# ShawnNew/Detectron2-CenterNet

Measured on AMD Instinct MI355X. Metric: images/sec at 512x512 (infer bs=64), higher is better.
Workload: dtype f16x3; 1 GPU; DLA-34 CenterNet eval forward+decode, 64x3x512x512 uint8 per GPU, 80 classes, K=100, random-init weights (BatchNorm statistics calibrated), DCN offsets ~N(0,1px), 100 detections per image post-processed; per_gpu_batch=64, global_batch=64, parallelism=replicas x1

## Files before the change

### detectron2-centernet_amd/csrc/conv_common.h

```cpp
#pragma once
#include "common.h"
#include <type_traits>
__device__ __forceinline__ int swz(int row) { return (0x78 >> (2 * ((row >> 2) & 3))) & 3; }

__device__ __forceinline__ bool tile_of_block(int nbx, int nby, int& m_tile, int& n_tile) {
  const int lin = blockIdx.x;
  const int xcd = lin & 7, sq = lin >> 3;
  const int mchunk = (nbx + 7) >> 3;
  n_tile = sq % nby;
  const int m_local = sq / nby;
  m_tile = xcd * mchunk + m_local;
  return m_local < mchunk && m_tile < nbx;
}

struct DcnSample {
  int off[4];
  float wt[4];
  float mask;
  f16 wm[4];
};

template <bool NM = false>
__device__ __forceinline__ void dcn_setup(const ConvArgs& a, bool row_ok, int pix_base, int hb, int wb,
                                          int tr, int ts, const float* omrow, DcnSample& sp) {
  sp.off[0] = sp.off[1] = sp.off[2] = sp.off[3] = -1;
// ... 95 lines not shown
#pragma unroll
        for (int j = 0; j < 4; ++j) { v0[j] = fmaxf(v0[j], 0.f); v1[j] = fmaxf(v1[j], 0.f); }
      } else if (a.act == CTDET_ACT_SIGMOID_CLAMP) {
#pragma unroll
        for (int j = 0; j < 4; ++j) {
          v0[j] = fminf(fmaxf(ctdet_sigmoid_exact(v0[j]), a.clamp_lo), a.clamp_hi);
          v1[j] = fminf(fmaxf(ctdet_sigmoid_exact(v1[j]), a.clamp_lo), a.clamp_hi);
        }
      }
      TOut* yp = (TOut*)a.y + (long)m * a.out_stride + c0;
      if constexpr (sizeof(TOut) == 2) {
        f16x8 o;
#pragma unroll
        for (int j = 0; j < 4; ++j) { o[j] = (f16)v0[j]; o[4 + j] = (f16)v1[j]; }
        *(f16x8*)yp = o;
      } else {
        *(f32x4*)yp = v0;
        *(f32x4*)(yp + 4) = v1;
      }
    }
  }
}

static __device__ __attribute__((aligned(16))) unsigned int g_zero_page[64];

template <int N>
__device__ __forceinline__ void wait_vmcnt() {
  asm volatile("s_waitcnt vmcnt(%0)" ::"n"(N) : "memory");
}

__device__ __forceinline__ void wait_lgkm0() { __builtin_amdgcn_s_waitcnt(0xC07F); }

__device__ __forceinline__ void gload2_sync(const float* p, float& v0, float& v1) {
  typedef float f32x2_ __attribute__((ext_vector_type(2)));
  f32x2_ v;
  asm volatile("global_load_dwordx2 %0, %1, off\n\ts_waitcnt vmcnt(0)" : "=&v"(v) : "v"(p) : "memory");
  v0 = v[0]; v1 = v[1];
}
__device__ __forceinline__ void gload4_sync_into(const float* p, f32x4& v) {
  asm volatile("global_load_dwordx4 %0, %1, off\n\ts_waitcnt vmcnt(0)" : "+v"(v) : "v"(p) : "memory");
}

__device__ __forceinline__ void dma16(const void* g, char* lds_wave_base) {
  const unsigned l = __builtin_amdgcn_readfirstlane((unsigned)(size_t)lds_wave_base);
  asm volatile("s_mov_b32 m0, %0\n\ts_nop 0\n\tglobal_load_lds_dwordx4 %1, off" ::"s"(l), "v"(g) : "memory", "m0");
}
// ... 51 lines not shown
```

### detectron2-centernet_amd/csrc/conv_f32.hip

```cpp
#include "conv_common.h"

template <int BP, int BC, int WP, int WC_, bool SP>
__global__ void __launch_bounds__(256) conv_f32_mfma_kernel(const ConvArgs a) {
  constexpr int KS = 16, EPV = 4;
  constexpr int TP = BP / WP / 16;
  constexpr int TC = BC / WC_ / 16;
  constexpr int A_LD = BP / 64;
  constexpr int BCL = BC < 64 ? 64 : BC;
  constexpr int B_LD = BCL / 64;
  constexpr int NLOAD = A_LD + B_LD;
  constexpr int STAGE = (BP + BCL) * 64;
  constexpr int NST = 3;
  static_assert(WP * WC_ == 4, "4 waves per workgroup");
  __shared__ __attribute__((aligned(16))) char smem[NST * STAGE];

  const int tid = threadIdx.x, lane = tid & 63;
  const int wave = __builtin_amdgcn_readfirstlane(tid >> 6);
  const int wp = wave / WC_, wc = wave % WC_;
  int m_tile, n_tile;
  if (!tile_of_block((a.M + BP - 1) / BP, a.Cout_pad / BC, m_tile, n_tile)) return;
  const int m0 = m_tile * BP, n0 = n_tile * BC;
  const float* __restrict__ x = (const float*)a.x;
  const float* __restrict__ w = (const float*)a.w;
  const float* zero = (const float*)g_zero_page;
// ... 104 lines not shown
    f32x4 wf[TC], pf[TP];
#pragma unroll
    for (int c = 0; c < TC; ++c) wf[c] = *(const f32x4*)(base + BP * 64 + (wc * 16 * TC + 16 * c) * 64 + frag_off);
#pragma unroll
    for (int p = 0; p < TP; ++p) pf[p] = *(const f32x4*)(base + (wp * 16 * TP + 16 * p) * 64 + frag_off);
    if constexpr (SP) {
#pragma unroll
      for (int p = 0; p < TP; ++p) mma_px<true, TC>(wf, pf[p], acc[p]);
    } else {
#pragma unroll
      for (int e = 0; e < 4; ++e)
#pragma unroll
        for (int p = 0; p < TP; ++p)
#pragma unroll
          for (int c = 0; c < TC; ++c)
            acc[p][c] = __builtin_amdgcn_mfma_f32_16x16x4f32(wf[c][e], pf[p][e], acc[p][c], 0, 0, 0);
    }
    st_c = st_c == NST - 1 ? 0 : st_c + 1;
    st_l = st_l == NST - 1 ? 0 : st_l + 1;
  }

  const int q = lane >> 4;
  const int cb = n0 + wc * 16 * TC;
#pragma unroll
  for (int p = 0; p < TP; ++p) {
    const int m = m0 + wp * 16 * TP + 16 * p + fr;
    if (m >= a.M) continue;
    epilogue_tiles<float, TC>(a, m, cb, q, acc[p]);
  }
}

template <int BP, int BC, int WP, int WC_, bool CAT, bool SP>
__global__ void __launch_bounds__(256, 2) conv_f32_uk_kernel(const ConvArgs a) {
  constexpr int KS = 16, EPV = 4;
  constexpr int TP = BP / WP / 16;
  constexpr int TC = BC / WC_ / 16;
  constexpr int A_LD = BP / 64;
  constexpr int BCL = BC < 64 ? 64 : BC;
  constexpr int B_LD = BCL / 64;
  constexpr int NLOAD = A_LD + B_LD;
  constexpr int STAGE = (BP + BCL) * 64;
  constexpr int NST = 3;
  static_assert(WP * WC_ == 4, "4 waves per workgroup");
  __shared__ __attribute__((aligned(16))) char smem[NST * STAGE];

  const int tid = threadIdx.x, lane = tid & 63;
  const int wave = __builtin_amdgcn_readfirstlane(tid >> 6);
  const int wp = wave / WC_, wc = wave % WC_;
  int m_tile, n_tile;
  if (!tile_of_block((a.M + BP - 1) / BP, a.Cout_pad / BC, m_tile, n_tile)) return;
  const int m0 = m_tile * BP, n0 = n_tile * BC;
  const float* zero = (const float*)g_zero_page;
// ... 101 lines not shown
    f32x4 wf[TC];
#pragma unroll
    for (int c = 0; c < TC; ++c) wf[c] = *(const f32x4*)(fragB + ST * STAGE + c * 1024);
#pragma unroll
    for (int p = 0; p < TP; ++p) {
      const f32x4 pf = *(const f32x4*)(fragA + ST * STAGE + p * 1024);
      mma_px<SP, TC>(wf, pf, acc[p]);
    }
  };
  using I0 = std::integral_constant<int, 0>;
  using I1 = std::integral_constant<int, 1>;
  using I2 = std::integral_constant<int, 2>;
  int kt = 0;
  for (; kt + 2 < nk; kt += 3) {
    kstep(kt, I0{}, I2{});
    kstep(kt + 1, I1{}, I0{});
    kstep(kt + 2, I2{}, I1{});
  }
  if (kt < nk) { kstep(kt, I0{}, I2{}); ++kt; }
  if (kt < nk) { kstep(kt, I1{}, I0{}); ++kt; }

  const int q = lane >> 4;
  const int cb = n0 + wc * 16 * TC;
#pragma unroll
  for (int p = 0; p < TP; ++p) {
    const int m = m0 + wp * 16 * TP + 16 * p + fr;
    if (m >= a.M) continue;
    epilogue_tiles<float, TC>(a, m, cb, q, acc[p]);
  }
}

template <int BP, int BC, int WP, int WC_, bool SP, bool NM = false>
__global__ void __launch_bounds__(256, 2) dcn_f32_mfma_kernel(const ConvArgs a) {
  constexpr int KS = 16, EPV = 4;
  constexpr int TP = BP / WP / 16;
  constexpr int TC = BC / WC_ / 16;
  constexpr int A_LD = BP / 64;
  constexpr int BCL = BC < 64 ? 64 : BC;
  constexpr int B_LD = BCL / 64;
  constexpr int ASTAGE = BP * 64, WSTAGE = BCL * 64;
  static_assert(WP * WC_ == 4, "4 waves per workgroup");
  __shared__ __attribute__((aligned(16))) char smem[2 * ASTAGE + 2 * WSTAGE];
  char* const smA = smem;
  char* const smW = smem + 2 * ASTAGE;

  const int tid = threadIdx.x, lane = tid & 63;
  const int wave = __builtin_amdgcn_readfirstlane(tid >> 6);
  const int wp = wave / WC_, wc = wave % WC_;
  int m_tile, n_tile;
  if (!tile_of_block((a.M + BP - 1) / BP, a.Cout_pad / BC, m_tile, n_tile)) return;
  const int m0 = m_tile * BP, n0 = n_tile * BC;
  const float* __restrict__ x = (const float*)a.x;
// ... 97 lines not shown
    const char* bW = smW + (kt & 1) * WSTAGE;
    f32x4 wf[TC], pf[TP];
#pragma unroll
    for (int c = 0; c < TC; ++c) wf[c] = *(const f32x4*)(bW + (wc * 16 * TC + 16 * c) * 64 + frag_off);
#pragma unroll
    for (int p = 0; p < TP; ++p) pf[p] = *(const f32x4*)(bA + (wp * 16 * TP + 16 * p) * 64 + frag_off);
    if constexpr (SP) {
#pragma unroll
      for (int p = 0; p < TP; ++p) mma_px<true, TC>(wf, pf[p], acc[p]);
    } else {
#pragma unroll
      for (int e = 0; e < 4; ++e)
#pragma unroll
        for (int p = 0; p < TP; ++p)
#pragma unroll
          for (int c = 0; c < TC; ++c)
            acc[p][c] = __builtin_amdgcn_mfma_f32_16x16x4f32(wf[c][e], pf[p][e], acc[p][c], 0, 0, 0);
    }
    if (more) blend_store(smA + ((kt + 1) & 1) * ASTAGE);
  }

  const int q = lane >> 4;
  const int cb = n0 + wc * 16 * TC;
#pragma unroll
  for (int p = 0; p < TP; ++p) {
    const int m = m0 + wp * 16 * TP + 16 * p + fr;
    if (m >= a.M) continue;
    epilogue_tiles<float, TC>(a, m, cb, q, acc[p]);
  }
}

template <int BC, bool SP, bool NM = false>
__global__ void __launch_bounds__(256, 2) dcn_f32_window_kernel(const ConvArgs a) {
  constexpr int TH = 8, TW = 16, BP = 128, MG = 4;
  constexpr int WR = TH + 2 + 2 * MG, WCOLS = TW + 2 + 2 * MG;
  constexpr int NPIECE = WR * WCOLS * 4;
  constexpr int W_LD = (NPIECE + 255) / 256;
  constexpr int WINB = ((NPIECE + 63) / 64) * 1024;
  constexpr int GEOB = 9 * BP * 16, GEOC = 9 * BP * 4;
  constexpr int TP = 2, TC = BC / 16;
  constexpr int B_LD = BC / 64, WST = BC * 64, NST = 2, STG = 3 * WST;
  static_assert(BC % 64 == 0 && WINB + GEOB + GEOC + NST * STG <= 81920, "two workgroups per CU");
  __shared__ __attribute__((aligned(16))) char smem[WINB + GEOB + GEOC + NST * STG];
  char* const win = smem;
  char* const geo = smem + WINB;
  char* const geoc = smem + WINB + GEOB;
  char* const ring = smem + WINB + GEOB + GEOC;

  const int tid = threadIdx.x, lane = tid & 63;
  const int wave = __builtin_amdgcn_readfirstlane(tid >> 6);
  const int tiles_x = a.W / TW, tiles_y = a.H / TH;
  int m_tile, n_tile;
// ... 171 lines not shown
      asm volatile("" ::: "memory");
      sample(0, chunk + 1, pfn);
    }
#pragma unroll
    for (int p = 0; p < TP; ++p) pf[p] = pfn[p];
    if (TS < 2) {
#pragma unroll
      for (int c = 0; c < TC; ++c) wf[c] = wfn[c];
    }
  };
  for (int chunk = 0; chunk < nch; ++chunk) {
    const int s = chunk * 3;
    tap(s, chunk, std::integral_constant<int, 0>{});
    tap(s, chunk, std::integral_constant<int, 1>{});
    tap(s, chunk, std::integral_constant<int, 2>{});
    tap(s + 1, chunk, std::integral_constant<int, 3>{});
    tap(s + 1, chunk, std::integral_constant<int, 4>{});
    tap(s + 1, chunk, std::integral_constant<int, 5>{});
    tap(s + 2, chunk, std::integral_constant<int, 6>{});
    tap(s + 2, chunk, std::integral_constant<int, 7>{});
    tap(s + 2, chunk, std::integral_constant<int, 8>{});
  }

#pragma unroll
  for (int p = 0; p < TP; ++p) {
    const int m = (b * a.H + ty0 + prow) * a.W + tx0 + 8 * p + pcol;
    epilogue_tiles<float, TC>(a, m, n0, q, acc[p]);
  }
}

template <int TP, int BC, bool COLS = false, bool NM = false, bool FUS = false>
__global__ void __launch_bounds__(512 / TP, (TP == 1 && BC == 64) ? 4 : 2) dcn_split_window_kernel(const ConvArgs a) {
  static_assert(!FUS || (TP == 2 && BC == 64 && !COLS && !NM), "the fused offset conv: inference form of the 64-cout DCNv2 tile");
  constexpr int TH = 8, TW = 16, BP = 128, MG = 4;
  constexpr int NT = 512 / TP;
  static_assert(BC * 4 <= NT, "at most one weight piece per thread and tap (waves beyond BC / 16 fetch none)");
  constexpr int WR = TH + 2 + 2 * MG, WCOLS = TW + 2 + 2 * MG;
  constexpr int NPIECE = WR * WCOLS * 4;
  constexpr int W_LD = (NPIECE + NT - 1) / NT;
  constexpr int WINB = ((NPIECE + 63) / 64) * 1024;
  constexpr int GEOW = 9 * BP * 16, GEOC = 9 * BP * 4;
  constexpr int TC = BC / 16;
  constexpr int WST = BC * 64, NST = 2, STG = 3 * WST;
  static_assert(WINB + GEOW + GEOC + NST * STG <= ((TP == 2 || BC == 64) ? 81920 : 163840), "two workgroups / one (128 couts) per CU");
  __shared__ __attribute__((aligned(16))) char smem[WINB + GEOW + GEOC + NST * STG];
  char* const win = smem;
  char* const geow = smem + WINB;
  char* const geoc = smem + WINB + GEOW;
  char* const ring = smem + WINB + GEOW + GEOC;

  const int tid = threadIdx.x, lane = tid & 63;
// ... 377 lines not shown
    if (T < 8) {
      blend(raw, b1, b2, T + 1, chunk);
    } else if (chunk + 1 < nch) {
      wait_vmcnt<0>();
      __builtin_amdgcn_s_barrier();
      asm volatile("" ::: "memory");
      gather(0, chunk + 1, raw);
      blend(raw, b1, b2, 0, chunk + 1);
    }
  };
  for (int chunk = 0; chunk < nch; ++chunk) {
    const int s = chunk * 3;
    tap(s, chunk, std::integral_constant<int, 0>{});
    tap(s, chunk, std::integral_constant<int, 1>{});
    tap(s, chunk, std::integral_constant<int, 2>{});
    tap(s + 1, chunk, std::integral_constant<int, 3>{});
    tap(s + 1, chunk, std::integral_constant<int, 4>{});
    tap(s + 1, chunk, std::integral_constant<int, 5>{});
    tap(s + 2, chunk, std::integral_constant<int, 6>{});
    tap(s + 2, chunk, std::integral_constant<int, 7>{});
    tap(s + 2, chunk, std::integral_constant<int, 8>{});
  }

#pragma unroll
  for (int p = 0; p < TP; ++p) {
    const int m = (b * a.H + ty0 + prow) * a.W + tx0 + (TP == 2 ? 8 * p : 0) + pcol;
    epilogue_tiles<float, TC>(a, m, n0, q, acc[p]);
  }
}

template <int R, int CIN, int TC, int STRIDE, int TH, bool NOCHECK, bool SP>
__global__ void __launch_bounds__(256) conv_f32_win_kernel(const ConvArgs a) {
  constexpr int TW = STRIDE == 1 ? 64 : 32;
  constexpr int WH = (TH - 1) * STRIDE + R, WW = (TW - 1) * STRIDE + R;
  constexpr int PB = CIN * 4;
  constexpr int PPR = WW * PB / 16;
  constexpr int NP = WH * PPR, ROUNDS = (NP + 255) / 256;
  constexpr int K = R * R * CIN, NK = (K + 15) / 16;
  constexpr int GPT = CIN / 4;
  constexpr int NT = TW / 16, RW = TH / 4;
  static_assert(TH % 4 == 0 && ROUNDS * 4096 <= 65536, "tile");
  __shared__ __attribute__((aligned(16))) char win[ROUNDS * 4096];

  const int tid = threadIdx.x, lane = tid & 63;
  const int wave = __builtin_amdgcn_readfirstlane(tid >> 6);
  const int fr = lane & 15, q = lane >> 4;
  const int tiles_x = a.Wo / TW, tiles_y = a.Ho / TH;
  const int tx0 = (blockIdx.x % tiles_x) * TW;
  const int ty0 = ((blockIdx.x / tiles_x) % tiles_y) * TH;
  const int b = blockIdx.x / (tiles_x * tiles_y);
  const float* zero = (const float*)g_zero_page;
// ... 72 lines not shown
        if constexpr (SP) {
          const f16x8 h0 = __builtin_bit_cast(f16x8, pf0), h1 = __builtin_bit_cast(f16x8, pf1);
#pragma unroll
          for (int c = 0; c < TC; ++c) {
            acc[0][c] = __builtin_amdgcn_mfma_f32_16x16x32_f16(wa[kt][c], h0, acc[0][c], 0, 0, 0);
            acc[1][c] = __builtin_amdgcn_mfma_f32_16x16x32_f16(wa[kt][c], h1, acc[1][c], 0, 0, 0);
          }
#pragma unroll
          for (int c = 0; c < TC; ++c) {
            acc[0][c] = __builtin_amdgcn_mfma_f32_16x16x32_f16(wb[kt][c], h0, acc[0][c], 0, 0, 0);
            acc[1][c] = __builtin_amdgcn_mfma_f32_16x16x32_f16(wb[kt][c], h1, acc[1][c], 0, 0, 0);
          }
        } else {
#pragma unroll
          for (int e = 0; e < 4; ++e)
#pragma unroll
            for (int c = 0; c < TC; ++c) {
              acc[0][c] = __builtin_amdgcn_mfma_f32_16x16x4f32(wf[kt][c][e], pf0[e], acc[0][c], 0, 0, 0);
              acc[1][c] = __builtin_amdgcn_mfma_f32_16x16x4f32(wf[kt][c][e], pf1[e], acc[1][c], 0, 0, 0);
            }
        }
      }
      const int m = (b * a.Ho + ty0 + wave * RW + rr) * a.Wo + tx0 + tc * 16 + fr;
      epilogue_tiles<float, TC>(a, m, 0, q, acc[0]);
      epilogue_tiles<float, TC>(a, m + 16, 0, q, acc[1]);
    }
  }
}

template <bool SP> static const char* sp_name() { return SP ? "f16x3" : "f32"; }

template <int R, int CIN, int TC, int STRIDE, int TH, bool SP>
static int launch_f32_win(const ConvArgs& a, hipStream_t s) {
  constexpr int TW = STRIDE == 1 ? 64 : 32;
  const int tiles = a.B * (a.Ho / TH) * (a.Wo / TW);
  CTDET_KERNEL("conv_%s_win_kernel<%dx%d,Cin%d,Cout%d,s%d>", sp_name<SP>(), R, R, CIN, 16 * TC, STRIDE);
  if (a.pad == 0)
    hipLaunchKernelGGL((conv_f32_win_kernel<R, CIN, TC, STRIDE, TH, true, SP>), dim3(tiles), dim3(256), 0, s, a);
  else
    hipLaunchKernelGGL((conv_f32_win_kernel<R, CIN, TC, STRIDE, TH, false, SP>), dim3(tiles), dim3(256), 0, s, a);
  CTDET_LAUNCH_CHECK();
  return 0;
}

template <bool DEFORM, bool SP, bool NM = false>
__global__ void __launch_bounds__(256) conv_direct_f32_kernel(const ConvArgs a) {
  const long idx = (long)blockIdx.x * 256 + threadIdx.x;
  const int CP = (a.Cout + 3) & ~3;
// ... 258 lines not shown
```

### detectron2-centernet_amd/csrc/conv_igemm.hip

```cpp
#include "common.h"
#include <type_traits>
#include <stdlib.h>

#include "conv_common.h"

template <int BP, int BC, int WP, int WC_, typename TOut>
__global__ void __launch_bounds__(256) conv_igemm_dma_kernel(const ConvArgs a) {
  constexpr int TP = BP / WP / 16;
  constexpr int TC = BC / WC_ / 16;
  constexpr int A_LD = BP / 64;
  constexpr int BCL = BC < 64 ? 64 : BC;
  constexpr int B_LD = BCL / 64;
  constexpr int NLOAD = A_LD + B_LD;
  constexpr int STAGE = (BP + BCL) * 64;
  constexpr int NST = 3;
  static_assert(WP * WC_ == 4, "4 waves per workgroup");
  __shared__ __attribute__((aligned(16))) char smem[NST * STAGE];

  const int tid = threadIdx.x, lane = tid & 63;
  const int wave = __builtin_amdgcn_readfirstlane(tid >> 6);
  const int wp = wave / WC_, wc = wave % WC_;
  int m_tile, n_tile;
  if (!tile_of_block((a.M + BP - 1) / BP, a.Cout_pad / BC, m_tile, n_tile)) return;
  const int m0 = m_tile * BP, n0 = n_tile * BC;
// ... 103 lines not shown

  int st_c = 0, st_l = 2;
  for (int kt = 0; kt < nk; ++kt) {
    if (kt + 1 < nk) wait_vmcnt<NLOAD>(); else wait_vmcnt<0>();
    asm volatile("s_waitcnt lgkmcnt(0)" ::: "memory");
    __builtin_amdgcn_s_barrier();
    if (kt + 2 < nk) { issue(kt + 2, st_l); advance_k(); }
    const char* base = smem + st_c * STAGE;
    f16x8 wf[TC];
#pragma unroll
    for (int c = 0; c < TC; ++c) wf[c] = *(const f16x8*)(base + BP * 64 + (wc * 16 * TC + 16 * c) * 64 + frag_off);
#pragma unroll
    for (int p = 0; p < TP; ++p) {
      const f16x8 pf = *(const f16x8*)(base + (wp * 16 * TP + 16 * p) * 64 + frag_off);
#pragma unroll
      for (int c = 0; c < TC; ++c) acc[p][c] = __builtin_amdgcn_mfma_f32_16x16x32_f16(wf[c], pf, acc[p][c], 0, 0, 0);
    }
    st_c = st_c == NST - 1 ? 0 : st_c + 1;
    st_l = st_l == NST - 1 ? 0 : st_l + 1;
  }

  const int q = lane >> 4;
  const int cb = n0 + wc * 16 * TC;
#pragma unroll
  for (int p = 0; p < TP; ++p) {
    const int m = m0 + wp * 16 * TP + 16 * p + fr;
    if (m >= a.M) continue;
    epilogue_tiles<TOut, TC>(a, m, cb, q, acc[p]);
  }
}

template <int BP, int BC, int WP, int WC_, bool CAT, typename TOut>
__global__ void __launch_bounds__(256, 2) conv_igemm_uk_kernel(const ConvArgs a) {
  constexpr int TP = BP / WP / 16;
  constexpr int TC = BC / WC_ / 16;
  constexpr int A_LD = BP / 64;
  constexpr int BCL = BC < 64 ? 64 : BC;
  constexpr int B_LD = BCL / 64;
  constexpr int NLOAD = A_LD + B_LD;
  constexpr int STAGE = (BP + BCL) * 64;
  constexpr int NST = 3;
  static_assert(WP * WC_ == 4, "4 waves per workgroup");
  __shared__ __attribute__((aligned(16))) char smem[NST * STAGE];

  const int tid = threadIdx.x, lane = tid & 63;
  const int wave = __builtin_amdgcn_readfirstlane(tid >> 6);
  const int wp = wave / WC_, wc = wave % WC_;
  int m_tile, n_tile;
  if (!tile_of_block((a.M + BP - 1) / BP, a.Cout_pad / BC, m_tile, n_tile)) return;
  const int m0 = m_tile * BP, n0 = n_tile * BC;
  const f16* zero = (const f16*)g_zero_page;
  asm volatile("" : "+v"(zero));
// ... 101 lines not shown
#pragma unroll
    for (int c = 0; c < TC; ++c) wf[c] = *(const f16x8*)(fragB + ST * STAGE + c * 1024);
#pragma unroll
    for (int p = 0; p < TP; ++p) {
      const f16x8 pf = *(const f16x8*)(fragA + ST * STAGE + p * 1024);
#pragma unroll
      for (int c = 0; c < TC; ++c) acc[p][c] = __builtin_amdgcn_mfma_f32_16x16x32_f16(wf[c], pf, acc[p][c], 0, 0, 0);
    }
  };
  using I0 = std::integral_constant<int, 0>;
  using I1 = std::integral_constant<int, 1>;
  using I2 = std::integral_constant<int, 2>;
  int kt = 0;
  for (; kt + 2 < nk; kt += 3) {
    kstep(kt, I0{}, I2{});
    kstep(kt + 1, I1{}, I0{});
    kstep(kt + 2, I2{}, I1{});
  }
  if (kt < nk) { kstep(kt, I0{}, I2{}); ++kt; }
  if (kt < nk) { kstep(kt, I1{}, I0{}); ++kt; }

  const int q = lane >> 4;
  const int cb = n0 + wc * 16 * TC;
#pragma unroll
  for (int p = 0; p < TP; ++p) {
    const int m = m0 + wp * 16 * TP + 16 * p + fr;
    if (m >= a.M) continue;
    epilogue_tiles<TOut, TC>(a, m, cb, q, acc[p]);
  }
}

template <int BC, int WP, int WC_, typename TOut, bool SP = false>
__global__ void __launch_bounds__(256, 2) conv3x3_halo_kernel(const ConvArgs a) {
  using TIn = std::conditional_t<SP, float, f16>;
  constexpr int CH = SP ? 16 : 32, EPV = SP ? 4 : 8;
  static_assert(!SP || std::is_same<TOut, float>::value, "split mode stores f32");
  constexpr int TH = 8, TW = 32, BP = TH * TW;
  constexpr int TP = BP / WP / 16;
  constexpr int TC = BC / WC_ / 16;
  constexpr int ROWS_W = TH / WP;
  constexpr int BCL = BC < 64 ? 64 : BC;
  constexpr int B_LD = BCL / 64;
  constexpr int HMAIN = 10 * 32 * 64, HSIDE = 4096, HBUF = HMAIN + HSIDE;
  constexpr int WST = BCL * 64;
  static_assert(WP * WC_ == 4 && TP == 2 * ROWS_W, "wave layout");
  __shared__ __attribute__((aligned(16))) char smem[2 * HBUF + 3 * WST];
  char* const ring = smem + 2 * HBUF;

  const int tid = threadIdx.x, lane = tid & 63;
  const int wave = __builtin_amdgcn_readfirstlane(tid >> 6);
  const int wp = wave / WC_, wc = wave % WC_;
  const int tiles_x = a.W / TW, tiles_y = a.H / TH;
// ... 107 lines not shown
      }
    }
  };
  auto chunk_steps = [&](int kt, int chunk, auto hbc) {
    kstep(kt + 0, chunk, std::integral_constant<int, 0>{}, hbc);
    kstep(kt + 1, chunk, std::integral_constant<int, 1>{}, hbc);
    kstep(kt + 2, chunk, std::integral_constant<int, 2>{}, hbc);
    kstep(kt + 3, chunk, std::integral_constant<int, 3>{}, hbc);
    kstep(kt + 4, chunk, std::integral_constant<int, 4>{}, hbc);
    kstep(kt + 5, chunk, std::integral_constant<int, 5>{}, hbc);
    kstep(kt + 6, chunk, std::integral_constant<int, 6>{}, hbc);
    kstep(kt + 7, chunk, std::integral_constant<int, 7>{}, hbc);
    kstep(kt + 8, chunk, std::integral_constant<int, 8>{}, hbc);
  };
  int chunk = 0;
  for (; chunk + 1 < nch; chunk += 2) {
    chunk_steps(chunk * 9, chunk, std::integral_constant<int, 0>{});
    chunk_steps(chunk * 9 + 9, chunk + 1, std::integral_constant<int, 1>{});
  }
  if (chunk < nch) chunk_steps(chunk * 9, chunk, std::integral_constant<int, 0>{});

  const int q = lane >> 4;
  const int cb = n0 + wc * 16 * TC;
#pragma unroll
  for (int p = 0; p < TP; ++p) {
    const int y = ty0 + row0 + (p >> 1), x = tx0 + 16 * (p & 1) + l15;
    const int m = (b * a.H + y) * a.W + x;
    epilogue_tiles<TOut, TC>(a, m, cb, q, acc[p]);
  }
}

template <int BC, int WP, int WC_, typename TOut, bool SP = false>
static int launch_halo(const ConvArgs& a, hipStream_t s) {
  const int nbx = a.B * (a.H / 8) * (a.W / 32), nby = a.Cout_pad / BC;
  dim3 grid(8 * ((nbx + 7) / 8) * nby);
  CTDET_KERNEL("conv3x3_halo_kernel<256x%d,%s>", BC, SP ? "f16x3" : out_name<TOut>());
  hipLaunchKernelGGL((conv3x3_halo_kernel<BC, WP, WC_, TOut, SP>), grid, dim3(256), 0, s, a);
  CTDET_LAUNCH_CHECK();
  return 0;
}

template <int BC, int WP, int WC_>
__global__ void __launch_bounds__(256, 2) conv3x3_halo_pair_kernel(const ConvArgs a) {
  constexpr int TH = 8, TW = 32, BP = TH * TW;
  constexpr int TP = BP / WP / 16;
  constexpr int TC = BC / WC_ / 16;
  constexpr int ROWS_W = TH / WP;
  constexpr int BCL = BC < 64 ? 64 : BC;
  constexpr int W_LD = BCL / 64;
  constexpr int HMAIN = 10 * 32 * 64, HSIDE = 4096, HBUF = HMAIN + HSIDE;
  constexpr int WIMG = BCL * 64, WST = 2 * WIMG, NST = 3;
  static_assert(WP * WC_ == 4 && TP == 2 * ROWS_W, "wave layout");
// ... 194 lines not shown
  };
  auto next_stage = [](int st) { return st == NST - 1 ? 0 : st + 1; };
  auto chunk_steps = [&](int chunk, int st0, auto hbc, auto p0c) {
    constexpr int P0 = decltype(p0c)::value;
    const int kt = chunk * 5;
    int st = st0;
    kstep(kt + 0, chunk, st, std::integral_constant<int, 0>{}, hbc, std::integral_constant<int, P0>{}); st = next_stage(st);
    kstep(kt + 1, chunk, st, std::integral_constant<int, 1>{}, hbc, std::integral_constant<int, P0 ^ 1>{}); st = next_stage(st);
    kstep(kt + 2, chunk, st, std::integral_constant<int, 2>{}, hbc, std::integral_constant<int, P0>{}); st = next_stage(st);
    kstep(kt + 3, chunk, st, std::integral_constant<int, 3>{}, hbc, std::integral_constant<int, P0 ^ 1>{}); st = next_stage(st);
    kstep(kt + 4, chunk, st, std::integral_constant<int, 4>{}, hbc, std::integral_constant<int, P0>{});
  };
  int chunk = 0, st0 = 0;
  for (; chunk + 1 < nch; chunk += 2) {
    chunk_steps(chunk, st0, std::integral_constant<int, 0>{}, std::integral_constant<int, 0>{});
    st0 = (st0 + 2) % 3;
    chunk_steps(chunk + 1, st0, std::integral_constant<int, 1>{}, std::integral_constant<int, 1>{});
    st0 = (st0 + 2) % 3;
  }
  if (chunk < nch) chunk_steps(chunk, st0, std::integral_constant<int, 0>{}, std::integral_constant<int, 0>{});

  const int q = lane >> 4;
  const int cb = n0 + wc * 16 * TC;
#pragma unroll
  for (int p = 0; p < TP; ++p) {
    const int y = ty0 + row0 + (p >> 1), x = tx0 + 16 * (p & 1) + l15;
    const int m = (b * a.H + y) * a.W + x;
    epilogue_tiles<float, TC>(a, m, cb, q, acc[p]);
  }
}

template <int BC>
constexpr int pair2_smem_bytes() {
  return 2 * (10 * 32 * 64 + 4096) + 3 * 2 * (BC < 64 ? 64 : BC) * 64;
}

template <int BC, int WP, int WC_, int TW>
__device__ __forceinline__ void pair2_kloop(const ConvArgs& a, char* smem, int b, int ty0, int tx0, int n0,
                                            f32x4 (&acc)[256 / WP / 16][BC / WC_ / 16]) {
  constexpr int TH = 256 / TW, BP = TH * TW;
  constexpr int EN = TW / 16;
  constexpr int RS = TW * 64;
  constexpr int RPR = 256 * 16 / RS;
  constexpr int TP = BP / WP / 16;
  constexpr int TC = BC / WC_ / 16;
  constexpr int ROWS_W = TH / WP;
  constexpr int BCL = BC < 64 ? 64 : BC;
  constexpr int W_LD = BCL / 64;
  constexpr int HMAIN = 10 * 32 * 64, HSIDE = 4096, HBUF = HMAIN + HSIDE;
  constexpr int WIMG = BCL * 64, WST = 2 * WIMG, NST = 3;
  static_assert(WP * WC_ == 4 && TP == EN * ROWS_W && (TH + 2 + RPR - 1) / RPR == 5, "wave layout");
  static_assert(2 * HBUF + NST * WST == pair2_smem_bytes<BC>(), "LDS layout");
// ... 203 lines not shown
    kstep(kt + 6, pair, std::integral_constant<int, 6>{});
    kstep(kt + 7, pair, std::integral_constant<int, 7>{});
    kstep(kt + 8, pair, std::integral_constant<int, 8>{});
  }
}

template <int BC, int WP, int WC_, int TW = 32>
__global__ void __launch_bounds__(256, BC > 64 ? 1 : 2) conv3x3_halo_pair2_kernel(const ConvArgs a) {
  constexpr int TH = 256 / TW, EN = TW / 16, TP = 256 / WP / 16, TC = BC / WC_ / 16, ROWS_W = TH / WP;
  __shared__ __attribute__((aligned(16))) char smem[pair2_smem_bytes<BC>()];
  const int tiles_x = a.W / TW, tiles_y = a.H / TH;
  int m_tile, n_tile;
  if (!tile_of_block(a.B * tiles_y * tiles_x, a.Cout_pad / BC, m_tile, n_tile)) return;
  const int tx0 = (m_tile % tiles_x) * TW;
  const int ty0 = ((m_tile / tiles_x) % tiles_y) * TH;
  const int b = m_tile / (tiles_x * tiles_y);
  const int n0 = n_tile * BC;
  f32x4 acc[TP][TC];
  pair2_kloop<BC, WP, WC_, TW>(a, smem, b, ty0, tx0, n0, acc);

  const int lane = threadIdx.x & 63, wave = __builtin_amdgcn_readfirstlane(threadIdx.x >> 6);
  const int row0 = (wave / WC_) * ROWS_W, l15 = lane & 15, q = lane >> 4;
  const int cb = n0 + (wave % WC_) * 16 * TC;
#pragma unroll
  for (int p = 0; p < TP; ++p) {
    const int y = ty0 + row0 + p / EN, x = tx0 + 16 * (p % EN) + l15;
    const int m = (b * a.H + y) * a.W + x;
    epilogue_tiles<float, TC>(a, m, cb, q, acc[p]);
  }
}

template <int BC, int WP, int WC_, typename TOut, int TW = 32>
__global__ void __launch_bounds__(256, 2) conv3x3_halo_tap2_kernel(const ConvArgs a) {
  constexpr int TH = 256 / TW, BP = TH * TW;
  constexpr int EN = TW / 16, RS = TW * 64, RPR = 256 * 16 / RS;
  constexpr int TP = BP / WP / 16;
  constexpr int TC = BC / WC_ / 16;
  constexpr int ROWS_W = TH / WP;
  constexpr int BCL = BC < 64 ? 64 : BC;
  constexpr int W_LD = BCL / 64;
  constexpr int HMAIN = 10 * 32 * 64, HSIDE = 4096, HBUF = HMAIN + HSIDE;
  constexpr int WIMG = BCL * 64, WST = 2 * WIMG, NST = 3;
  static_assert(WP * WC_ == 4 && TP == EN * ROWS_W && (TH + 2 + RPR - 1) / RPR == 5, "wave layout");
  static_assert(2 * HBUF + NST * WST <= 81920, "two workgroups per CU");
  __shared__ __attribute__((aligned(16))) char smem[2 * HBUF + NST * WST];
  char* const ring = smem + 2 * HBUF;

  const int tid = threadIdx.x, lane = tid & 63;
  const int wave = __builtin_amdgcn_readfirstlane(tid >> 6);
  const int wp = wave / WC_, wc = wave % WC_;
  const int tiles_x = a.W / TW, tiles_y = a.H / TH;
  int m_tile, n_tile;
// ... 161 lines not shown
#pragma unroll
      for (int i = 2 * sl; i < 2 * sl + 2; ++i) mfma1(Par{}, 2, i, 1, 0);
      __builtin_amdgcn_sched_barrier(0);
    }
    load_px1(2, NextS{}, 0);
    load_px1(3, NextS{}, 0);
    __builtin_amdgcn_sched_barrier(0);
  };
  for (int pair = 0; pair < npair; ++pair) {
    const int kt = pair * 9;
    kstep(kt + 0, pair, std::integral_constant<int, 0>{});
    kstep(kt + 1, pair, std::integral_constant<int, 1>{});
    kstep(kt + 2, pair, std::integral_constant<int, 2>{});
    kstep(kt + 3, pair, std::integral_constant<int, 3>{});
    kstep(kt + 4, pair, std::integral_constant<int, 4>{});
    kstep(kt + 5, pair, std::integral_constant<int, 5>{});
    kstep(kt + 6, pair, std::integral_constant<int, 6>{});
    kstep(kt + 7, pair, std::integral_constant<int, 7>{});
    kstep(kt + 8, pair, std::integral_constant<int, 8>{});
  }

  const int q = lane >> 4;
  const int cb = n0 + wc * 16 * TC;
#pragma unroll
  for (int p = 0; p < TP; ++p) {
    const int y = ty0 + row0 + p / EN, x = tx0 + 16 * (p % EN) + l15;
    const int m = (b * a.H + y) * a.W + x;
    epilogue_tiles<TOut, TC>(a, m, cb, q, acc[p]);
  }
}

template <int BC, int WP, int WC_>
static int launch_halo_pair_t(const ConvArgs& a, hipStream_t s) {
  const int nbx = a.B * (a.H / 8) * (a.W / 32), nby = a.Cout_pad / BC;
  dim3 grid(8 * ((nbx + 7) / 8) * nby);
  CTDET_KERNEL("conv3x3_halo_pair_kernel<256x%d,f16x3>", BC);
  hipLaunchKernelGGL((conv3x3_halo_pair_kernel<BC, WP, WC_>), grid, dim3(256), 0, s, a);
  CTDET_LAUNCH_CHECK();
  return 0;
}

template <int BC, int WP, int WC_, int TW = 32>
static int launch_halo_pair2_t(const ConvArgs& a, hipStream_t s) {
  const int nbx = a.B * (a.H / (256 / TW)) * (a.W / TW), nby = a.Cout_pad / BC;
  dim3 grid(8 * ((nbx + 7) / 8) * nby);
  CTDET_KERNEL(TW == 32 ? "conv3x3_halo_pair2_kernel<256x%d,f16x3>" : "conv3x3_halo_pair2_kernel<16x16x%d,f16x3>", BC);
  hipLaunchKernelGGL((conv3x3_halo_pair2_kernel<BC, WP, WC_, TW>), grid, dim3(256), 0, s, a);
  CTDET_LAUNCH_CHECK();
  return 0;
}

template <int BC, int WP, int WC_, typename TOut, int TW = 32>
// ... 287 lines not shown
    pair2_kloop<BC, WP, 1, TW>(c, smem, b, ty0, tx0, n0, acc);

    f16x8 hf[TP][TC / 2], lf[TP][TC / 2];
#pragma unroll
    for (int hb = 0; hb < TC / 2; ++hb) {
      const int c0 = n0 + hb * 32 + q * 8;
      const f32x4 sa = *(const f32x4*)(a.s1 + c0), sb = *(const f32x4*)(a.s1 + c0 + 4);
      const f32x4 ba = *(const f32x4*)(a.b1 + c0), bb = *(const f32x4*)(a.b1 + c0 + 4);
#pragma unroll
      for (int p = 0; p < TP; ++p) {
        const f32x4 v0 = acc[p][2 * hb] * sa + ba, v1 = acc[p][2 * hb + 1] * sb + bb;
        f16x8 hi, lo;
#pragma unroll
        for (int j = 0; j < 8; ++j) {
          const float h = fmaxf(j < 4 ? v0[j] : v1[j - 4], 0.f);
          hi[j] = (f16)h;
          lo[j] = (f16)(h - (float)hi[j]);
        }
        hf[p][hb] = hi;
        lf[p][hb] = lo;
      }
    }
    for (int ot = 0; ot < ntile2; ++ot) {
      f32x4 o[TP];
#pragma unroll
      for (int p = 0; p < TP; ++p) o[p] = (f32x4){0.f, 0.f, 0.f, 0.f};
      const f16* wrow = w2 + (long)(ot * 16 + l15) * (2 * HID) + sl * BC + q * 8;
#pragma unroll
      for (int hb = 0; hb < TC / 2; ++hb) {
        const f16x8 X = *(const f16x8*)(wrow + hb * 32), Y = *(const f16x8*)(wrow + HID + hb * 32);
#pragma unroll
        for (int p = 0; p < TP; ++p) o[p] = __builtin_amdgcn_mfma_f32_16x16x32_f16(X, hf[p][hb], o[p], 0, 0, 0);
#pragma unroll
        for (int p = 0; p < TP; ++p) o[p] = __builtin_amdgcn_mfma_f32_16x16x32_f16(Y, hf[p][hb], o[p], 0, 0, 0);
#pragma unroll
        for (int p = 0; p < TP; ++p) o[p] = __builtin_amdgcn_mfma_f32_16x16x32_f16(X, lf[p][hb], o[p], 0, 0, 0);
      }
      const int c0 = ot * 16 + 4 * q;
      if (c0 < cw) {
#pragma unroll
        for (int p = 0; p < TP; ++p) {
          float* yp = yh + mpix[p] * ystride + c0;
          f32x4 v = o[p];
          if (sl > 0) v = *(const f32x4*)yp + v;
          if (sl == NSL - 1) {
            v = v * *(const f32x4*)(b2 + rows2 + c0) + *(const f32x4*)(b2 + c0);
            if (act == CTDET_ACT_RELU) {
#pragma unroll
              for (int j = 0; j < 4; ++j) v[j] = fmaxf(v[j], 0.f);
            } else if (act == CTDET_ACT_SIGMOID_CLAMP) {
#pragma unroll
              for (int j = 0; j < 4; ++j) v[j] = fminf(fmaxf(ctdet_sigmoid_exact(v[j]), a.clamp_lo), a.clamp_hi);
            }
          }
          *(f32x4*)yp = v;
        }
      }
    }
  }
}

int launch_head_fused_x3(const HeadArgs& a, hipStream_t s) {
  CTDET_CHECK(a.nheads >= 1 && a.nheads <= 4, "head_fused_x3: 1..4 heads");
  CTDET_CHECK(head_fused_x_ok(a, true) && (((size_t)a.w1 | (size_t)a.s1 | (size_t)a.b1) & 15) == 0,
              "head_fused_x3: needs Cin %% 32 == 0 and a map divisible by 8x32 or 16x16 (Cin=%d, %dx%d)", a.Cin, a.H, a.W);
  for (int h = 0; h < a.nheads; ++h)
    CTDET_CHECK(a.cout[h] >= 1 && a.cout[h] <= 256 && a.y_stride[h] % 4 == 0 && a.y_stride[h] >= ((a.cout[h] + 3) & ~3) &&
                    ((((size_t)a.y[h]) | (size_t)a.w2[h] | (size_t)a.b2[h]) & 15) == 0,
                "head_fused_x3: head %d: bad output (cout %d, stride %d)", h, a.cout[h], a.y_stride[h]);
// ... 1126 lines not shown
  for (int c = 0; c < TC; ++c) {
    const f16* wr = (const f16*)a.w + (long)cout_of<TC>(c, fr >> 2, fr & 3) * a.Kpad + q * 8;
#pragma unroll
    for (int kt = 0; kt < NK; ++kt) wf[kt][c] = *(const f16x8*)(wr + kt * 32);
  }
  int kaddr[NK];
#pragma unroll
  for (int kt = 0; kt < NK; ++kt) {
    const int G = kt * 4 + q;
    const int tap = G / GPT;
    const bool tail = tap >= R * R;
    const int tr = tail ? 0 : tap / R, ts = tail ? 0 : tap - (tap / R) * R;
    kaddr[kt] = ((wave * RW * STRIDE + tr) * WW + fr * STRIDE + ts) * PB + (tail ? 0 : (G - tap * GPT) * 16);
  }
  wait_vmcnt<0>();
  __syncthreads();

#pragma unroll
  for (int rr = 0; rr < RW; ++rr) {
#pragma unroll
    for (int tc = 0; tc < NT; ++tc) {
      constexpr int dummy = 0; (void)dummy;
      const int toff = (rr * STRIDE * WW + tc * 16 * STRIDE) * PB;
      f32x4 acc[TC];
#pragma unroll
      for (int c = 0; c < TC; ++c) acc[c] = (f32x4){0.f, 0.f, 0.f, 0.f};
#pragma unroll
      for (int kt = 0; kt < NK; ++kt) {
        const f16x8 pf = *(const f16x8*)(win + kaddr[kt] + toff);
#pragma unroll
        for (int c = 0; c < TC; ++c) acc[c] = __builtin_amdgcn_mfma_f32_16x16x32_f16(wf[kt][c], pf, acc[c], 0, 0, 0);
      }
      const int m = (b * a.Ho + ty0 + wave * RW + rr) * a.Wo + tx0 + tc * 16 + fr;
      epilogue_tiles<TOut, TC>(a, m, 0, q, acc);
    }
  }
}

template <int R, int CIN, int TC, int STRIDE, typename TOut>
static int launch_win(const ConvArgs& a, hipStream_t s) {
  constexpr int TH = STRIDE == 1 ? 16 : 8, TW = STRIDE == 1 ? 64 : 32;
  const int blocks = a.B * (a.Ho / TH) * (a.Wo / TW);
  CTDET_KERNEL("conv_win_kernel<%dx%d,Cin%d,Cout%d,s%d,%s>", R, R, CIN, 16 * TC, STRIDE, out_name<TOut>());
  if (a.pad == 0)
    hipLaunchKernelGGL((conv_win_kernel<R, CIN, TC, STRIDE, true, TOut>), dim3(blocks), dim3(256), 0, s, a);
  else
    hipLaunchKernelGGL((conv_win_kernel<R, CIN, TC, STRIDE, false, TOut>), dim3(blocks), dim3(256), 0, s, a);
  CTDET_LAUNCH_CHECK();
  return 0;
}



template <int BP, int BC, int WP, int WC_, typename TOut>
static int launch_dma(const ConvArgs& a, hipStream_t s) {
  const int nbx = (a.M + BP - 1) / BP, nby = a.Cout_pad / BC;
  dim3 grid(8 * ((nbx + 7) / 8) * nby);
// ... 122 lines not shown
```

Measured before the change: 4475 images/s.

## Batch conv epilogue loads per wave and prefetch head partial sums before MFMA

Adds a wave-level epilogue that groups output tiles into batches, first issuing scale, bias and residual loads for a batch and then applying them and storing 16-byte vectors. It replaces the per-tile epilogue in the implicit-GEMM, DCN and window conv kernels. In the fused head kernel it also loads the previous partial sums and scale/bias before the MFMA loop so their latency overlaps compute. The intent is to hide global-load latency in the epilogue, at the cost of higher register pressure and more template complexity.

```diff
diff --git a/detectron2-centernet_amd/csrc/conv_common.h b/detectron2-centernet_amd/csrc/conv_common.h
--- a/detectron2-centernet_amd/csrc/conv_common.h
+++ b/detectron2-centernet_amd/csrc/conv_common.h
@@ -1,6 +1,7 @@
 #pragma once
 #include "common.h"
 #include <type_traits>
+#include <utility>
 __device__ __forceinline__ int swz(int row) { return (0x78 >> (2 * ((row >> 2) & 3))) & 3; }
 
 __device__ __forceinline__ bool tile_of_block(int nbx, int nby, int& m_tile, int& n_tile) {
@@ -142,6 +143,155 @@
   }
 }
 
+template <int... I, typename F>
+__device__ __forceinline__ void static_for_seq(std::integer_sequence<int, I...>, F&& f) { (f(std::integral_constant<int, I>{}), ...); }
+template <int N, typename F>
+__device__ __forceinline__ void static_for(F&& f) { static_for_seq(std::make_integer_sequence<int, N>{}, f); }
+
+template <int TP, int TC>
+constexpr int epilogue_batch() { return TP * TC >= 32 ? 2 : TP * (TC / 2); }
+template <int BP, int TP, int TC, bool ACC_AGPR = false>
+constexpr int epilogue_batch_tiled() {
+  constexpr int whole = TP * (TC / 2);
+  if (ACC_AGPR) return BP == 128 ? 0 : (whole < 2 ? whole : 2);
+  if (TP * TC >= 32 || (BP == 128 && TP * TC >= 16)) return 2;
+  return whole < 8 ? whole : 8;
+}
+
+template <typename TOut, int TP, int TC, bool GUARD = false, int NB = epilogue_batch<TP, TC>()>
+__device__ __forceinline__ void epilogue_wave(const ConvArgs& a, const int (&m)[TP], int cbase, int q,
+                                              const f32x4 (&acc)[TP][TC]) {
+  constexpr int VEC = 16 / sizeof(TOut);
+  bool batched = false;
+  if constexpr (TC % 2 == 0 && NB > 0)
+    batched = (a.out_stride % VEC) == 0 && (((size_t)a.y) & 15) == 0 &&
+              (!a.res || ((a.res_stride % VEC) == 0 && (((size_t)a.res) & 15) == 0)) && cbase + 16 * TC <= a.Cout;
+  if (NB == 0 || !batched) {
+#pragma unroll
+    for (int p = 0; p < TP; ++p)
+      if (!GUARD || m[p] >= 0) epilogue_tiles<TOut, TC>(a, m[p], cbase, q, acc[p]);
+    return;
+  }
+  if constexpr (TC % 2 == 0 && NB > 0) {
+#pragma clang fp contract(off)
+    constexpr int NG = TP * (TC / 2), NBATCH = NG / NB;
+    constexpr int HB = NB > TP ? NB / TP : 1;
+    constexpr int RV = sizeof(TOut) == 2 ? 1 : 2;
+    static_assert(NG % NB == 0 && (NB % TP == 0 || TP % NB == 0), "batch size");
+    const bool has_s = a.scale != nullptr, has_b = a.bias != nullptr, has_r = a.res != nullptr;
+    const int cw0 = cbase + q * 8;
+    f32x4 sc[HB][2], bi[HB][2], rr[NB][RV];
+    int cw = cw0, mb[TP];
+    auto issue = [&](auto kc) {
+      constexpr int k = decltype(kc)::value, h0 = k * NB / TP;
+      asm volatile("" : "+v"(cw) :: "memory");
+#pragma unroll
+      for (int j = 0; j < (NB < TP ? NB : TP); ++j) {
+        const int p = (k * NB + j) % TP;
+        mb[p] = m[p];
+        asm volatile("" : "+v"(mb[p]));
+      }
+      if (has_s) {
+#pragma unroll
+        for (int hl = 0; hl < HB; ++hl) {
+          sc[hl][0] = *(const f32x4*)(a.scale + cw + (h0 + hl) * 32);
+          sc[hl][1] = *(const f32x4*)(a.scale + cw + (h0 + hl) * 32 + 4);
+        }
+      }
+      if (has_b) {
+#pragma unroll
+        for (int hl = 0; hl < HB; ++hl) {
+          bi[hl][0] = *(const f32x4*)(a.bias + cw + (h0 + hl) * 32);
+          bi[hl][1] = *(const f32x4*)(a.bias + cw + (h0 + hl) * 32 + 4);
+        }
+      }
+      if (has_r) {
+#pragma unroll
+        for (int j = 0; j < NB; ++j) {
+          constexpr int g0 = k * NB;
+          const int p = (g0 + j) % TP, h = (g0 + j) / TP;
+          const int mm = (GUARD && mb[p] < 0) ? 0 : mb[p];
+          const TOut* rp = (const TOut*)a.res + (long)mm * a.res_stride + cw + h * 32;
+          rr[j][0] = *(const f32x4*)rp;
+          if constexpr (RV == 2) rr[j][1] = *(const f32x4*)(rp + 4);
+        }
+      }
+    };
+    auto finish = [&](auto kc) {
+      constexpr int k = decltype(kc)::value, g0 = k * NB, h0 = g0 / TP;
+      f32x4 v[NB][2];
+#pragma unroll
+      for (int j = 0; j < NB; ++j) {
+        const int p = (g0 + j) % TP, h = (g0 + j) / TP;
+        v[j][0] = acc[p][2 * h];
+        v[j][1] = acc[p][2 * h + 1];
+      }
+      if (has_s) {
+#pragma unroll
+        for (int j = 0; j < NB; ++j) {
+          const int hl = (g0 + j) / TP - h0;
+          v[j][0] = v[j][0] * sc[hl][0];
+          v[j][1] = v[j][1] * sc[hl][1];
+        }
+      }
+      if (has_b) {
+#pragma unroll
+        for (int j = 0; j < NB; ++j) {
+          const int hl = (g0 + j) / TP - h0;
+          v[j][0] = v[j][0] + bi[hl][0];
+          v[j][1] = v[j][1] + bi[hl][1];
+        }
+      }
+      if (has_r) {
+#pragma unroll
+        for (int j = 0; j < NB; ++j) {
+          if constexpr (sizeof(TOut) == 2) {
+            const f16x8 r = __builtin_bit_cast(f16x8, rr[j][0]);
+#pragma unroll
+            for (int i = 0; i < 4; ++i) { v[j][0][i] += (float)r[i]; v[j][1][i] += (float)r[4 + i]; }
+          } else {
+            v[j][0] = v[j][0] + rr[j][0];
+            v[j][1] = v[j][1] + rr[j][RV - 1];
+          }
+        }
+      }
+      if (a.act == CTDET_ACT_RELU) {
+#pragma unroll
+        for (int j = 0; j < NB; ++j)
+#pragma unroll
+          for (int i = 0; i < 4; ++i) { v[j][0][i] = fmaxf(v[j][0][i], 0.f); v[j][1][i] = fmaxf(v[j][1][i], 0.f); }
+      } else if (a.act == CTDET_ACT_SIGMOID_CLAMP) {
+#pragma unroll
+        for (int j = 0; j < NB; ++j)
+#pragma unroll
+          for (int i = 0; i < 4; ++i) {
+            v[j][0][i] = fminf(fmaxf(ctdet_sigmoid_exact(v[j][0][i]), a.clamp_lo), a.clamp_hi);
+            v[j][1][i] = fminf(fmaxf(ctdet_sigmoid_exact(v[j][1][i]), a.clamp_lo), a.clamp_hi);
+          }
+      }
+#pragma unroll
+      for (int j = 0; j < NB; ++j) {
+        const int p = (g0 + j) % TP, h = (g0 + j) / TP;
+        if (GUARD && mb[p] < 0) continue;
+        TOut* yp = (TOut*)a.y + (long)mb[p] * a.out_stride + cw + h * 32;
+        if constexpr (sizeof(TOut) == 2) {
+          f16x8 o;
+#pragma unroll
+          for (int i = 0; i < 4; ++i) { o[i] = (f16)v[j][0][i]; o[4 + i] = (f16)v[j][1][i]; }
+          *(f16x8*)yp = o;
+        } else {
+          *(f32x4*)yp = v[j][0];
+          *(f32x4*)(yp + 4) = v[j][1];
+        }
+      }
+    };
+    static_for<NBATCH>([&](auto kc) {
+      issue(kc);
+      finish(kc);
+    });
+  }
+}
+
 static __device__ __attribute__((aligned(16))) unsigned int g_zero_page[64];
 
 template <int N>
diff --git a/detectron2-centernet_amd/csrc/conv_f32.hip b/detectron2-centernet_amd/csrc/conv_f32.hip
--- a/detectron2-centernet_amd/csrc/conv_f32.hip
+++ b/detectron2-centernet_amd/csrc/conv_f32.hip
@@ -150,12 +150,13 @@
 
   const int q = lane >> 4;
   const int cb = n0 + wc * 16 * TC;
+  int mo[TP];
 #pragma unroll
   for (int p = 0; p < TP; ++p) {
     const int m = m0 + wp * 16 * TP + 16 * p + fr;
-    if (m >= a.M) continue;
-    epilogue_tiles<float, TC>(a, m, cb, q, acc[p]);
-  }
+    mo[p] = m < a.M ? m : -1;
+  }
+  epilogue_wave<float, TP, TC, true, epilogue_batch_tiled<BP, TP, TC, true>()>(a, mo, cb, q, acc);
 }
 
 template <int BP, int BC, int WP, int WC_, bool CAT, bool SP>
@@ -303,12 +304,13 @@
 
   const int q = lane >> 4;
   const int cb = n0 + wc * 16 * TC;
+  int mo[TP];
 #pragma unroll
   for (int p = 0; p < TP; ++p) {
     const int m = m0 + wp * 16 * TP + 16 * p + fr;
-    if (m >= a.M) continue;
-    epilogue_tiles<float, TC>(a, m, cb, q, acc[p]);
-  }
+    mo[p] = m < a.M ? m : -1;
+  }
+  epilogue_wave<float, TP, TC, true, epilogue_batch_tiled<BP, TP, TC>()>(a, mo, cb, q, acc);
 }
 
 template <int BP, int BC, int WP, int WC_, bool SP, bool NM = false>
@@ -452,12 +454,13 @@
 
   const int q = lane >> 4;
   const int cb = n0 + wc * 16 * TC;
+  int mo[TP];
 #pragma unroll
   for (int p = 0; p < TP; ++p) {
     const int m = m0 + wp * 16 * TP + 16 * p + fr;
-    if (m >= a.M) continue;
-    epilogue_tiles<float, TC>(a, m, cb, q, acc[p]);
-  }
+    mo[p] = m < a.M ? m : -1;
+  }
+  epilogue_wave<float, TP, TC, true, epilogue_batch_tiled<BP, TP, TC>()>(a, mo, cb, q, acc);
 }
 
 template <int BC, bool SP, bool NM = false>
@@ -675,11 +678,12 @@
     tap(s + 2, chunk, std::integral_constant<int, 8>{});
   }
 
+  int mo[TP];
 #pragma unroll
   for (int p = 0; p < TP; ++p) {
-    const int m = (b * a.H + ty0 + prow) * a.W + tx0 + 8 * p + pcol;
-    epilogue_tiles<float, TC>(a, m, n0, q, acc[p]);
-  }
+    mo[p] = (b * a.H + ty0 + prow) * a.W + tx0 + 8 * p + pcol;
+  }
+  epilogue_wave<float, TP, TC>(a, mo, n0, q, acc);
 }
 
 template <int TP, int BC, bool COLS = false, bool NM = false, bool FUS = false>
@@ -1103,11 +1107,12 @@
     tap(s + 2, chunk, std::integral_constant<int, 8>{});
   }
 
+  int mo[TP];
 #pragma unroll
   for (int p = 0; p < TP; ++p) {
-    const int m = (b * a.H + ty0 + prow) * a.W + tx0 + (TP == 2 ? 8 * p : 0) + pcol;
-    epilogue_tiles<float, TC>(a, m, n0, q, acc[p]);
-  }
+    mo[p] = (b * a.H + ty0 + prow) * a.W + tx0 + (TP == 2 ? 8 * p : 0) + pcol;
+  }
+  epilogue_wave<float, TP, TC>(a, mo, n0, q, acc);
 }
 
 template <int R, int CIN, int TC, int STRIDE, int TH, bool NOCHECK, bool SP>
@@ -1226,8 +1231,8 @@
         }
       }
       const int m = (b * a.Ho + ty0 + wave * RW + rr) * a.Wo + tx0 + tc * 16 + fr;
-      epilogue_tiles<float, TC>(a, m, 0, q, acc[0]);
-      epilogue_tiles<float, TC>(a, m + 16, 0, q, acc[1]);
+      const int mo[2] = {m, m + 16};
+      epilogue_wave<float, 2, TC>(a, mo, 0, q, acc);
     }
   }
 }
diff --git a/detectron2-centernet_amd/csrc/conv_igemm.hip b/detectron2-centernet_amd/csrc/conv_igemm.hip
--- a/detectron2-centernet_amd/csrc/conv_igemm.hip
+++ b/detectron2-centernet_amd/csrc/conv_igemm.hip
@@ -149,12 +149,13 @@
 
   const int q = lane >> 4;
   const int cb = n0 + wc * 16 * TC;
+  int mo[TP];
 #pragma unroll
   for (int p = 0; p < TP; ++p) {
     const int m = m0 + wp * 16 * TP + 16 * p + fr;
-    if (m >= a.M) continue;
-    epilogue_tiles<TOut, TC>(a, m, cb, q, acc[p]);
-  }
+    mo[p] = m < a.M ? m : -1;
+  }
+  epilogue_wave<TOut, TP, TC, true, epilogue_batch_tiled<BP, TP, TC, true>()>(a, mo, cb, q, acc);
 }
 
 template <int BP, int BC, int WP, int WC_, bool CAT, typename TOut>
@@ -302,12 +303,13 @@
 
   const int q = lane >> 4;
   const int cb = n0 + wc * 16 * TC;
+  int mo[TP];
 #pragma unroll
   for (int p = 0; p < TP; ++p) {
     const int m = m0 + wp * 16 * TP + 16 * p + fr;
-    if (m >= a.M) continue;
-    epilogue_tiles<TOut, TC>(a, m, cb, q, acc[p]);
-  }
+    mo[p] = m < a.M ? m : -1;
+  }
+  epilogue_wave<TOut, TP, TC, true, epilogue_batch_tiled<BP, TP, TC>()>(a, mo, cb, q, acc);
 }
 
 template <int BC, int WP, int WC_, typename TOut, bool SP = false>
@@ -461,12 +463,13 @@
 
   const int q = lane >> 4;
   const int cb = n0 + wc * 16 * TC;
+  int mo[TP];
 #pragma unroll
   for (int p = 0; p < TP; ++p) {
     const int y = ty0 + row0 + (p >> 1), x = tx0 + 16 * (p & 1) + l15;
-    const int m = (b * a.H + y) * a.W + x;
-    epilogue_tiles<TOut, TC>(a, m, cb, q, acc[p]);
-  }
+    mo[p] = (b * a.H + y) * a.W + x;
+  }
+  epilogue_wave<TOut, TP, TC>(a, mo, cb, q, acc);
 }
 
 template <int BC, int WP, int WC_, typename TOut, bool SP = false>
@@ -707,12 +710,13 @@
 
   const int q = lane >> 4;
   const int cb = n0 + wc * 16 * TC;
+  int mo[TP];
 #pragma unroll
   for (int p = 0; p < TP; ++p) {
     const int y = ty0 + row0 + (p >> 1), x = tx0 + 16 * (p & 1) + l15;
-    const int m = (b * a.H + y) * a.W + x;
-    epilogue_tiles<float, TC>(a, m, cb, q, acc[p]);
-  }
+    mo[p] = (b * a.H + y) * a.W + x;
+  }
+  epilogue_wave<float, TP, TC>(a, mo, cb, q, acc);
 }
 
 template <int BC>
@@ -962,12 +966,13 @@
   const int lane = threadIdx.x & 63, wave = __builtin_amdgcn_readfirstlane(threadIdx.x >> 6);
   const int row0 = (wave / WC_) * ROWS_W, l15 = lane & 15, q = lane >> 4;
   const int cb = n0 + (wave % WC_) * 16 * TC;
+  int mo[TP];
 #pragma unroll
   for (int p = 0; p < TP; ++p) {
     const int y = ty0 + row0 + p / EN, x = tx0 + 16 * (p % EN) + l15;
-    const int m = (b * a.H + y) * a.W + x;
-    epilogue_tiles<float, TC>(a, m, cb, q, acc[p]);
-  }
+    mo[p] = (b * a.H + y) * a.W + x;
+  }
+  epilogue_wave<float, TP, TC>(a, mo, cb, q, acc);
 }
 
 template <int BC, int WP, int WC_, typename TOut, int TW = 32>
@@ -1175,12 +1180,13 @@
 
   const int q = lane >> 4;
   const int cb = n0 + wc * 16 * TC;
+  int mo[TP];
 #pragma unroll
   for (int p = 0; p < TP; ++p) {
     const int y = ty0 + row0 + p / EN, x = tx0 + 16 * (p % EN) + l15;
-    const int m = (b * a.H + y) * a.W + x;
-    epilogue_tiles<TOut, TC>(a, m, cb, q, acc[p]);
-  }
+    mo[p] = (b * a.H + y) * a.W + x;
+  }
+  epilogue_wave<TOut, TP, TC>(a, mo, cb, q, acc);
 }
 
 template <int BC, int WP, int WC_>
@@ -1514,6 +1520,16 @@
       }
     }
     for (int ot = 0; ot < ntile2; ++ot) {
+      const int c0 = ot * 16 + 4 * q;
+      const bool live = c0 < cw;
+      f32x4 prev[TP] = {}, s2 = {}, bias2 = {};
+      if (live) {
+        if (sl > 0) {
+#pragma unroll
+          for (int p = 0; p < TP; ++p) prev[p] = *(const f32x4*)(yh + mpix[p] * ystride + c0);
+        }
+        if (sl == NSL - 1) { s2 = *(const f32x4*)(b2 + rows2 + c0); bias2 = *(const f32x4*)(b2 + c0); }
+      }
       f32x4 o[TP];
 #pragma unroll
       for (int p = 0; p < TP; ++p) o[p] = (f32x4){0.f, 0.f, 0.f, 0.f};
@@ -1528,15 +1544,14 @@
 #pragma unroll
         for (int p = 0; p < TP; ++p) o[p] = __builtin_amdgcn_mfma_f32_16x16x32_f16(X, lf[p][hb], o[p], 0, 0, 0);
       }
-      const int c0 = ot * 16 + 4 * q;
-      if (c0 < cw) {
+      if (live) {
 #pragma unroll
         for (int p = 0; p < TP; ++p) {
           float* yp = yh + mpix[p] * ystride + c0;
           f32x4 v = o[p];
-          if (sl > 0) v = *(const f32x4*)yp + v;
+          if (sl > 0) v = prev[p] + v;
           if (sl == NSL - 1) {
-            v = v * *(const f32x4*)(b2 + rows2 + c0) + *(const f32x4*)(b2 + c0);
+            v = v * s2 + bias2;
             if (act == CTDET_ACT_RELU) {
 #pragma unroll
               for (int j = 0; j < 4; ++j) v[j] = fmaxf(v[j], 0.f);
@@ -2709,17 +2724,17 @@
     for (int tc = 0; tc < NT; ++tc) {
       constexpr int dummy = 0; (void)dummy;
       const int toff = (rr * STRIDE * WW + tc * 16 * STRIDE) * PB;
-      f32x4 acc[TC];
-#pragma unroll
-      for (int c = 0; c < TC; ++c) acc[c] = (f32x4){0.f, 0.f, 0.f, 0.f};
+      f32x4 acc[1][TC];
+#pragma unroll
+      for (int c = 0; c < TC; ++c) acc[0][c] = (f32x4){0.f, 0.f, 0.f, 0.f};
 #pragma unroll
       for (int kt = 0; kt < NK; ++kt) {
         const f16x8 pf = *(const f16x8*)(win + kaddr[kt] + toff);
 #pragma unroll
-        for (int c = 0; c < TC; ++c) acc[c] = __builtin_amdgcn_mfma_f32_16x16x32_f16(wf[kt][c], pf, acc[c], 0, 0, 0);
-      }
-      const int m = (b * a.Ho + ty0 + wave * RW + rr) * a.Wo + tx0 + tc * 16 + fr;
-      epilogue_tiles<TOut, TC>(a, m, 0, q, acc);
+        for (int c = 0; c < TC; ++c) acc[0][c] = __builtin_amdgcn_mfma_f32_16x16x32_f16(wf[kt][c], pf, acc[0][c], 0, 0, 0);
+      }
+      const int mo[1] = {(b * a.Ho + ty0 + wave * RW + rr) * a.Wo + tx0 + tc * 16 + fr};
+      epilogue_wave<TOut, 1, TC>(a, mo, 0, q, acc);
     }
   }
 }
```

After: 4564 images/s (median of 6 runs). 2.0% higher.
